# jrkerns/pylinac

Hardware: AMD Instinct MI355X
Metric: EPID images/s, filter->threshold->profile->peak on 1024^2 batch (higher is better)
Workload: dtype f64

## Files before the change

### pylinac_amd/csrc/gaussian_mm.hip

```cpp
#include <type_traits>

#include "pl_common.h"

namespace {

constexpr int kMmHalo = 24;
constexpr int kMmMaxRad = 24;

typedef int v4i __attribute__((ext_vector_type(4)));

constexpr int kMmDigits = 5;
constexpr int kMmQ = 40;

struct MmParams {
  unsigned band[kMmDigits][4][24];
  int c1;
  int c4;
  int radius;
  double wd[kMmMaxRad + 1];
};

bool mm_make_params(const double* h_wts , int R, MmParams& p) {
  if (R < 1 || R > kMmMaxRad) return false;
  double wmax = 0.0, W = 0.0;
  for (int k = 0; k <= 2 * R; ++k) {
    if (!(h_wts[k] >= 0.0)) return false;
    wmax = h_wts[k] > wmax ? h_wts[k] : wmax;
    W += h_wts[k];
  }
  if (!(wmax > 0.0) || !(W < 2.0)) return false;
  constexpr int Q = kMmQ;
  if (__builtin_ldexp(wmax, Q) >= 5.0e11) return false;
  long long wq[2 * kMmMaxRad + 1];
  long long WQ = 0;
  double eq = 0.0;
  signed char dig[kMmDigits][kMmMaxRad + 1];
  for (int k = 0; k <= 2 * R; ++k) {
    wq[k] = (long long)__builtin_llround(__builtin_ldexp(h_wts[k], Q));
    WQ += wq[k];
    eq += __builtin_fabs(h_wts[k] - __builtin_ldexp((double)wq[k], -Q));
  }
  for (int j = 0; j <= R; ++j) {
    if (wq[R - j] != wq[R + j]) return false;
    long long v = wq[R - j];
    for (int d = 0; d < kMmDigits; ++d) {
      const long long lo = ((v + 128) & 255) - 128;
      dig[d][j] = (signed char)lo;
      v = (v - lo) >> 8;
    }
    if (v != 0) return false;
  }
  for (int d = 0; d < kMmDigits; ++d)
    for (int c = 0; c < 4; ++c) {
      unsigned char bytes[96];
      for (int x = 0; x < 96; ++x) {
        const int pidx = x + c - 39;
        const int dist = pidx < 0 ? -pidx : pidx;
        bytes[x] = dist <= R ? (unsigned char)dig[d][dist] : 0;
      }
      for (int q = 0; q < 24; ++q)
        p.band[d][c][q] = (unsigned)bytes[4 * q] | ((unsigned)bytes[4 * q + 1] << 8) | ((unsigned)bytes[4 * q + 2] << 16) |
                          ((unsigned)bytes[4 * q + 3] << 24);
    }
  const double D = __builtin_ldexp(65535.0 * eq * (1.0 + 1e-9) + 65536.0 * __builtin_fabs(W - 1.0) + 1e-9, Q) +
                   (double)(2 * R + 1) * 16384.0 + 256.0;
  constexpr long long M = 1LL << 23;
  if (!(D < (double)M)) return false;
  const long long C = 32896LL * WQ + M;
  p.c1 = (int)((C & 0xffffffffLL) >> 8);
  p.c4 = (int)(C >> 32);
  p.radius = R;
  for (int j = 0; j <= kMmMaxRad; ++j) p.wd[j] = j <= R ? h_wts[R - j] : 0.0;
  return true;
}

__device__ __forceinline__ v4i mm_band_operand(const MmParams& P, int d, int lane) {
  const int p0 = 16 * (lane >> 4) - (lane & 15) + 15;
  const unsigned* src = &P.band[d][p0 & 3][p0 >> 2];
  return v4i{(int)src[0], (int)src[1], (int)src[2], (int)src[3]};
}

template <typename F>
__device__ __forceinline__ double mm_exact(F raw , const MmParams& P) {
  const int R = P.radius;
  double a = raw(0) * P.wd[0];
  for (int j = R; j >= 1; --j) a = __builtin_fma(raw(-j) + raw(j), P.wd[j], a);
  const double off = __builtin_fabs(__builtin_amdgcn_fract(__builtin_fabs(a)) - 0.5);
  if (off > 0.5 - 4e-9) {
    a = raw(0) * P.wd[0];
    for (int j = R; j >= 1; --j) a = a + (raw(-j) + raw(j)) * P.wd[j];
  }
  return a;
}

struct MmAcc { v4i v, z; };

struct MmConst { v4i c1, c4; };
__device__ __forceinline__ MmConst mm_const(const MmParams& P) {
  return MmConst{v4i{P.c1, P.c1, P.c1, P.c1}, v4i{P.c4, P.c4, P.c4, P.c4}};
}

template <bool IMG_IS_A>
__device__ __forceinline__ MmAcc mm_tile(v4i img_lo, v4i img_hi, const v4i (&w)[kMmDigits], const MmConst& K) {
  auto mm = [&](v4i img, v4i band, v4i c) -> v4i {
    return IMG_IS_A ? __builtin_amdgcn_mfma_i32_16x16x64_i8(img, band, c, 0, 0, 0)
                    : __builtin_amdgcn_mfma_i32_16x16x64_i8(band, img, c, 0, 0, 0);
  };
  v4i t = mm(img_lo, w[1], K.c1);
  t = mm(img_hi, w[0], t);
  t = mm(img_lo, w[2], t >> 8);
  t = mm(img_hi, w[1], t);
  v4i t3 = mm(img_lo, w[3], t >> 8);
  t3 = mm(img_hi, w[2], t3);
  v4i t4 = mm(img_lo, w[4], (t3 >> 8) + K.c4);
  t4 = mm(img_hi, w[3], t4);
  MmAcc r;
  r.v = mm(img_hi, w[4], t4 >> 8);
  r.z = (t3 | t4) & 255;
  return r;
}

template <bool IMG_IS_A, int NT>
__device__ __forceinline__ void mm_tiles(const v4i (&lo)[NT], const v4i (&hi)[NT], const v4i (&w)[kMmDigits], const MmConst& K,
                                         MmAcc (&r)[NT]) {
  auto mm = [&](v4i img, v4i band, v4i c) -> v4i {
    return IMG_IS_A ? __builtin_amdgcn_mfma_i32_16x16x64_i8(img, band, c, 0, 0, 0)
                    : __builtin_amdgcn_mfma_i32_16x16x64_i8(band, img, c, 0, 0, 0);
  };
  v4i t[NT], t3[NT], t4[NT];
#pragma unroll
  for (int i = 0; i < NT; ++i) t[i] = mm(lo[i], w[1], K.c1);
#pragma unroll
  for (int i = 0; i < NT; ++i) t[i] = mm(hi[i], w[0], t[i]);
#pragma unroll
  for (int i = 0; i < NT; ++i) t[i] = mm(lo[i], w[2], t[i] >> 8);
#pragma unroll
  for (int i = 0; i < NT; ++i) t[i] = mm(hi[i], w[1], t[i]);
#pragma unroll
  for (int i = 0; i < NT; ++i) t3[i] = mm(lo[i], w[3], t[i] >> 8);
#pragma unroll
  for (int i = 0; i < NT; ++i) t3[i] = mm(hi[i], w[2], t3[i]);
#pragma unroll
  for (int i = 0; i < NT; ++i) t4[i] = mm(lo[i], w[4], (t3[i] >> 8) + K.c4);
#pragma unroll
  for (int i = 0; i < NT; ++i) t4[i] = mm(hi[i], w[3], t4[i]);
#pragma unroll
  for (int i = 0; i < NT; ++i) {
    r[i].v = mm(hi[i], w[4], t4[i] >> 8);
    r[i].z = (t3[i] | t4[i]) & 255;
  }
}

template <bool SIGNED>
__device__ __forceinline__ double mm_value(unsigned char lo, unsigned char hi) {
  const int x = ((int)(signed char)hi + 128) * 256 + ((int)(signed char)lo + 128);
  return (double)(x - (SIGNED ? 32768 : 0));
}

constexpr int kFCols = 256;
constexpr int kFWin = kFCols + 2 * kMmHalo;
constexpr int kFPlane = kFWin * 16;
constexpr int kFQuadPitch = (kFWin / 4) * 16;

__device__ __forceinline__ int f_cell(int c) { return kFQuadPitch * (c & 3) + 16 * (c >> 2); }

struct FQuad { uint2 r[4]; };

__device__ __forceinline__ uint4 f_ldsq(const unsigned char* p) {
  return *reinterpret_cast<const uint4*>(p);
}

__device__ __forceinline__ void mm_set(uint2& res, int q, unsigned v16) {
  unsigned d = q < 2 ? res.x : res.y;
  d = (q & 1) ? (d & 0x0000ffffu) | (v16 << 16) : (d & 0xffff0000u) | v16;
  if (q < 2) res.x = d; else res.y = d;
}

__device__ __forceinline__ bool mm_wave_flat(const uint4& lo, const uint4& hi) {
  const unsigned l0 = lo.x, h0 = hi.x;
  const unsigned lf = __builtin_amdgcn_readfirstlane(l0), hf = __builtin_amdgcn_readfirstlane(h0);
  const unsigned d = (lo.y ^ l0) | (lo.z ^ l0) | (lo.w ^ l0) | (hi.y ^ h0) | (hi.z ^ h0) | (hi.w ^ h0) |
                     (__builtin_amdgcn_alignbit(l0, l0, 8) ^ l0) | (__builtin_amdgcn_alignbit(h0, h0, 8) ^ h0) | (lf ^ l0) | (hf ^ h0);
  return __ballot(d != 0u) == 0ull;
}

template <bool SIGNED>
__device__ __forceinline__ uint2 mm_finish_flag(const MmAcc& r, bool& bad) {
  unsigned v[4], z[4];
#pragma unroll
  for (int q = 0; q < 4; ++q) {
    v[q] = (unsigned)r.v[q];
    z[q] = (unsigned)r.z[q];
    if (SIGNED) v[q] = (v[q] + (v[q] < 32768u ? 1u : 0u)) ^ 0x8000u;
  }
  unsigned zm = z[0] < z[1] ? z[0] : z[1];
  zm = zm < z[2] ? zm : z[2];
  zm = zm < z[3] ? zm : z[3];
  bad = zm == 0u;
  return uint2{__builtin_amdgcn_perm(v[1], v[0], 0x05040100u), __builtin_amdgcn_perm(v[3], v[2], 0x05040100u)};
}

constexpr int kGThreads = 512;
constexpr int kGWaves = kGThreads / PL_WAVE;
constexpr int kGSlots = 5;
constexpr int kGInLo = 0;
constexpr int kGInHi = kGInLo + kGSlots * kFPlane;
constexpr int kGVLo = kGInHi + kGSlots * kFPlane;
constexpr int kGVHi = kGVLo + 2 * kFPlane;
constexpr int kGLds = kGVHi + 2 * kFPlane;

template <typename T>
__global__ void __launch_bounds__(kGThreads) __attribute__((amdgpu_waves_per_eu(4, 4)))
gauss2d_mm(const T* __restrict__ in, T* __restrict__ out, int h, int w, int strips, int segs, int seg_rows, const MmParams P) {
  constexpr bool kSigned = (T)-1 < (T)0;
  constexpr unsigned kHiFlip = kSigned ? 0u : 0x80808080u;
  __shared__ __attribute__((aligned(16))) unsigned char s_mem[kGLds];

  unsigned id = pl_xcd_remap(blockIdx.x, gridDim.x);
  const int ct = id % strips;
  id /= strips;
  const int rt = id % segs;
  const size_t frame = id / segs;
  const int tid = threadIdx.x;
  const int lane = tid & (PL_WAVE - 1);
  const int wave = __builtin_amdgcn_readfirstlane(tid / PL_WAVE);
  const int j = lane & 15, g = lane >> 4;
  const int c0 = ct * kFCols, r_begin = rt * seg_rows;
  const int r_end = r_begin + seg_rows < h ? r_begin + seg_rows : h;
  const int nsteps = (r_end - r_begin + 15) / 16;
  if (nsteps <= 0) return;
  const T* f = in + frame * (size_t)h * w;
  const int wcols = w - c0 < kFCols ? w - c0 : kFCols;
  const int nht = (wcols + 15) / 16;
  const int nvt = nht + 3;
  const bool ragged = (wcols & 15) != 0;
  const __amdgpu_buffer_rsrc_t src = pl_make_rsrc_bounded(f, (unsigned)h * (unsigned)w * 2u);
  const __amdgpu_buffer_rsrc_t dstb = pl_make_rsrc_bounded(out + (frame * (size_t)h + r_begin) * w, (unsigned)(r_end - r_begin) * (unsigned)w * 2u);

  const int rq = g;
  const int cqx = wave < 4 ? 16 * wave + j : 64 + j;
  const bool loader = (wave < 4 || (wave == 4 && j < 12)) && 4 * cqx < 16 * nvt;
  const int col0 = c0 - kMmHalo + 4 * cqx;
  const bool mir = col0 < 0 || col0 >= w;
  const int mc = col0 < 0 ? -col0 - 4 : (col0 >= w ? 2 * w - 4 - col0 : col0);
  const bool across = col0 < w && col0 + 4 > w;
  const unsigned colb = 2u * (unsigned)mc;
  const unsigned colb_ld = across ? colb - 4u : colb;
  const int qd0 = 16 * cqx + 4 * rq + (mir ? 3 * kFQuadPitch : 0);
  const int qdstep = mir ? -kFQuadPitch : kFQuadPitch;
  const unsigned wb = 2u * (unsigned)w;
  auto load_quad = [&](int k, FQuad& x) {
    const int rbase = r_begin - kMmHalo + 16 * k + 4 * rq;
#pragma unroll
    for (int i = 0; i < 4; ++i) {
      int r = rbase + i;
      r ^= r >> 31;
      const int r2 = 2 * h - 1 - r;
      r = r < r2 ? r : r2;
      x.r[i] = pl_buffer_load_u64(src, loader ? (unsigned)r * wb + colb_ld : 0x80000000u, 0);
    }
  };
  const bool any_across = (w & 3) == 2;
  auto store_quad = [&](int slot, const FQuad& xin) {
    if (!loader) return;
    FQuad x = xin;
    if (any_across) {
#pragma unroll
      for (int i = 0; i < 4; ++i) {
        const unsigned up = xin.r[i].y;
        x.r[i].x = across ? up : xin.r[i].x;
        x.r[i].y = across ? __builtin_amdgcn_alignbit(up, up, 16) : up;
      }
    }
    unsigned char* base = s_mem + kGInLo + slot * kFPlane + qd0;
#pragma unroll
    for (int half = 0; half < 2; ++half) {
      const unsigned a0 = half ? x.r[0].y : x.r[0].x, a1 = half ? x.r[1].y : x.r[1].x;
      const unsigned a2 = half ? x.r[2].y : x.r[2].x, a3 = half ? x.r[3].y : x.r[3].x;
      const unsigned e0 = __builtin_amdgcn_perm(a1, a0, 0x05010400u);
      const unsigned e1 = __builtin_amdgcn_perm(a3, a2, 0x05010400u);
      const unsigned o0 = __builtin_amdgcn_perm(a1, a0, 0x07030602u);
      const unsigned o1 = __builtin_amdgcn_perm(a3, a2, 0x07030602u);
      unsigned char* pe = base + (2 * half) * qdstep;
      unsigned char* po = base + (2 * half + 1) * qdstep;
      *reinterpret_cast<unsigned*>(pe) = __builtin_amdgcn_perm(e1, e0, 0x05040100u) ^ 0x80808080u;
      *reinterpret_cast<unsigned*>(pe + (kGInHi - kGInLo)) = __builtin_amdgcn_perm(e1, e0, 0x07060302u) ^ kHiFlip;
      *reinterpret_cast<unsigned*>(po) = __builtin_amdgcn_perm(o1, o0, 0x05040100u) ^ 0x80808080u;
      *reinterpret_cast<unsigned*>(po + (kGInHi - kGInLo)) = __builtin_amdgcn_perm(o1, o0, 0x07060302u) ^ kHiFlip;
    }
  };
  v4i band[kMmDigits];
#pragma unroll
  for (int d = 0; d < kMmDigits; ++d) band[d] = mm_band_operand(P, d, lane);
  __builtin_amdgcn_s_waitcnt(0x0f70);
  MmConst K = mm_const(P);
  asm volatile("" : "+v"(K.c1), "+v"(K.c4));
  FQuad nxt;
  {
    FQuad a[4];
#pragma unroll
    for (int k = 0; k < 4; ++k) load_quad(k, a[k]);
    load_quad(4, nxt);
#pragma unroll
    for (int k = 0; k < 4; ++k) store_quad(k, a[k]);
  }
  __syncthreads();

  const int lane_cell = f_cell(j);
  int slot_g = g;
  int wslot = 4;
  auto step = [&](int s) {
    const int vb = (s & 1) * kFPlane;
    const int lrow = 16 * s + j;
    const bool row_ok = r_begin + lrow < r_end;

    {
      const unsigned char* ain = s_mem + kGInLo + slot_g * kFPlane + lane_cell;
      unsigned char* vout = s_mem + kGVLo + vb + 16 * j + 4 * g;
      auto run = [&](auto NT, int t0, int tstep) {
        constexpr int N = decltype(NT)::value;
        auto tile_of = [&](int i) { const int t = t0 + tstep * i; return t < nvt ? t : 0; };
        unsigned badbits = 0;
        v4i lo[N], hi[N];
#pragma unroll
        for (int i = 0; i < N; ++i) {
          const uint4 qlo = f_ldsq(ain + 64 * tile_of(i));
          const uint4 qhi = f_ldsq(ain + 64 * tile_of(i) + (kGInHi - kGInLo));
          lo[i] = v4i{(int)qlo.x, (int)qlo.y, (int)qlo.z, (int)qlo.w};
          hi[i] = v4i{(int)qhi.x, (int)qhi.y, (int)qhi.z, (int)qhi.w};
        }
        MmAcc acc[N];
        mm_tiles<true, N>(lo, hi, band, K, acc);
#pragma unroll
        for (int i = 0; i < N; ++i) {
          bool bad;
          const uint2 res = mm_finish_flag<kSigned>(acc[i], bad);
          badbits |= (bad && row_ok) ? (1u << i) : 0u;
          unsigned char* vd = vout + 256 * tile_of(i);
          *reinterpret_cast<unsigned*>(vd) = __builtin_amdgcn_perm(res.y, res.x, 0x06040200u) ^ 0x80808080u;
          *reinterpret_cast<unsigned*>(vd + (kGVHi - kGVLo)) = __builtin_amdgcn_perm(res.y, res.x, 0x07050301u) ^ kHiFlip;
        }
        if (__ballot(badbits != 0u) == 0ull) return;
        auto sample = [&](int x, int p) {
          const int a = ((s + (p >> 4)) % kGSlots) * kFPlane + f_cell(x) + (p & 15);
          return mm_value<kSigned>(s_mem[kGInLo + a], s_mem[kGInHi + a]);
        };
#pragma unroll 1
        for (int i = 0; i < N; ++i) {
          if (__ballot((badbits >> i) & 1u) == 0ull) continue;
          const int t = tile_of(i);
          unsigned char* vd = vout + 256 * t;
          const uint4 flo = *reinterpret_cast<const uint4*>(ain + 64 * t);
          const uint4 fhi = *reinterpret_cast<const uint4*>(ain + 64 * t + (kGInHi - kGInLo));
          if (mm_wave_flat(flo, fhi)) {
            const double c = sample(16 * t, 0);
            const unsigned v = (unsigned short)pl_from_double<T>(mm_exact([&](int) { return c; }, P));
            *reinterpret_cast<unsigned*>(vd) = (0x01010101u * (v & 255u)) ^ 0x80808080u;
            *reinterpret_cast<unsigned*>(vd + (kGVHi - kGVLo)) = (0x01010101u * (v >> 8)) ^ kHiFlip;
          } else {
            const MmAcc ra = mm_tile<true>(v4i{(int)flo.x, (int)flo.y, (int)flo.z, (int)flo.w}, v4i{(int)fhi.x, (int)fhi.y, (int)fhi.z, (int)fhi.w}, band, K);
            if ((badbits >> i) & 1u) {
#pragma unroll 1
              for (int q = 0; q < 4; ++q) {
                if (ra.z[q] != 0) continue;
                const int x = 16 * t + 4 * g + q;
                const unsigned v = (unsigned short)pl_from_double<T>(mm_exact([&](int k) { return sample(x, kMmHalo + j + k); }, P));
                vd[q] = (unsigned char)((v & 255u) ^ 0x80u);
                vd[q + (kGVHi - kGVLo)] = (unsigned char)((v >> 8) ^ (kHiFlip & 0x80u));
              }
            }
          }
        }
      };
      if (wave < 5) run(std::integral_constant<int, 2>{}, wave, 5); else run(std::integral_constant<int, 3>{}, 5 + wave, 3);
    }
    store_quad(wslot, nxt);
    load_quad(s + 5, nxt);
    __syncthreads();

    {
      const unsigned char* bin = s_mem + kGVLo + vb + 16 * j + 256 * g;
      const unsigned doff = row_ok ? ((unsigned)lrow * (unsigned)w + (unsigned)(c0 + 4 * g)) * 2u : 0x80000000u;
      const unsigned doff16 = row_ok ? ((unsigned)lrow * (unsigned)w + (unsigned)(c0 + 8 * (g >> 1))) * 2u : 0x80000000u;
      auto store_cut = [&](unsigned off, int x0, unsigned d0, unsigned d1, unsigned d2, unsigned d3) {
        const unsigned d[4] = {d0, d1, d2, d3};
#pragma unroll
        for (int k = 0; k < 4; ++k) pl_buffer_store_u32(d[k], dstb, x0 + 2 * k < wcols ? off + 4u * (unsigned)k : 0x80000000u, 0);
      };
      auto tile_of = [&](int i) { const int t = 2 * wave + i; return t < nht ? t : 0; };
      constexpr int N = 2;
      unsigned badbits = 0;
      auto hpass = [&](auto RAGGED) {
        v4i lo[N], hi[N];
#pragma unroll
        for (int i = 0; i < N; ++i) {
          const uint4 qlo = f_ldsq(bin + 256 * tile_of(i));
          const uint4 qhi = f_ldsq(bin + 256 * tile_of(i) + (kGVHi - kGVLo));
          lo[i] = v4i{(int)qlo.x, (int)qlo.y, (int)qlo.z, (int)qlo.w};
          hi[i] = v4i{(int)qhi.x, (int)qhi.y, (int)qhi.z, (int)qhi.w};
        }
        MmAcc acc[N];
        mm_tiles<false, N>(lo, hi, band, K, acc);
        bool bad0, bad1;
        const uint2 r0 = mm_finish_flag<kSigned>(acc[0], bad0), r1 = mm_finish_flag<kSigned>(acc[1], bad1);
        badbits |= ((bad0 && row_ok) ? 1u : 0u) | ((bad1 && row_ok) ? 2u : 0u);
        const auto sx = __builtin_amdgcn_permlane16_swap(r0.x, r1.x, false, false);
        const auto sy = __builtin_amdgcn_permlane16_swap(r0.y, r1.y, false, false);
        const unsigned tsel = (g & 1) ? (unsigned)tile_of(1) : (unsigned)tile_of(0);
        const uint4 piece{(unsigned)sx[0], (unsigned)sy[0], (unsigned)sx[1], (unsigned)sy[1]};
        if (!decltype(RAGGED)::value) {
          pl_buffer_store_u128(piece, dstb, doff16 + 32u * tsel, 0);
        } else {
          store_cut(doff16 + 32u * tsel, 16 * (int)tsel + 8 * (g >> 1), piece.x, piece.y, piece.z, piece.w);
        }
      };
      if (ragged) hpass(std::true_type{}); else hpass(std::false_type{});
      if (__ballot(badbits != 0u) != 0ull) {
        __builtin_amdgcn_s_waitcnt(0x0f70);
        auto store_cut2 = [&](unsigned off, int x0, unsigned d0, unsigned d1) {
          pl_buffer_store_u32(d0, dstb, x0 < wcols ? off : 0x80000000u, 0);
          pl_buffer_store_u32(d1, dstb, x0 + 2 < wcols ? off + 4u : 0x80000000u, 0);
        };
        auto sample = [&](int row, int x) {
          const int a = vb + 256 * (x >> 4) + 16 * row + (x & 15);
          return mm_value<kSigned>(s_mem[kGVLo + a], s_mem[kGVHi + a]);
        };
#pragma unroll 1
        for (int i = 0; i < N; ++i) {
          if (__ballot((badbits >> i) & 1u) == 0ull) continue;
          const int t = tile_of(i);
          const uint4 flo = *reinterpret_cast<const uint4*>(bin + 256 * t);
          const uint4 fhi = *reinterpret_cast<const uint4*>(bin + 256 * t + (kGVHi - kGVLo));
          if (mm_wave_flat(flo, fhi)) {
            const double c = sample(0, 16 * t);
            const unsigned v = (unsigned short)pl_from_double<T>(mm_exact([&](int) { return c; }, P));
            store_cut2(doff + 32u * (unsigned)t, 16 * t + 4 * g, v | (v << 16), v | (v << 16));
          } else {
            const MmAcc ra = mm_tile<false>(v4i{(int)flo.x, (int)flo.y, (int)flo.z, (int)flo.w}, v4i{(int)fhi.x, (int)fhi.y, (int)fhi.z, (int)fhi.w}, band, K);
            if ((badbits >> i) & 1u) {
              bool dummy;
              uint2 res = mm_finish_flag<kSigned>(ra, dummy);
#pragma unroll 1
              for (int q = 0; q < 4; ++q) {
                if (ra.z[q] != 0) continue;
                const int x = kMmHalo + 16 * t + 4 * g + q;
                mm_set(res, q, (unsigned short)pl_from_double<T>(mm_exact([&](int k) { return sample(j, x + k); }, P)));
              }
              store_cut2(doff + 32u * (unsigned)t, 16 * t + 4 * g, res.x, res.y);
            }
          }
        }
      }
    }
    slot_g = slot_g == kGSlots - 1 ? 0 : slot_g + 1;
    wslot = wslot == kGSlots - 1 ? 0 : wslot + 1;
  };
#pragma unroll 1
  for (int s = 0; s < nsteps; ++s) step(s);
}


template <typename T>
int launch_mm2d_t(const T* in, T* out, int64_t n, int h, int w, const MmParams& P, hipStream_t st) {
  const int strips = (int)pl_cdiv(w, kFCols);
  const int64_t resident = (int64_t)pl_cu_count() * 2;
  const int64_t max_segs = h / 128 > 1 ? h / 128 : 1;
  int64_t segs = 1, best = -1;
  for (int64_t cand = 1; cand <= max_segs; ++cand) {
    const int64_t rows = pl_cdiv(pl_cdiv(h, cand), 16) * 16;
    const int64_t wgs = n * strips * pl_cdiv(h, rows);
    const int64_t cost = pl_cdiv(wgs, resident) * (rows / 16 + 3);
    if (best < 0 || cost < best) { best = cost; segs = cand; }
  }
  const int seg_rows = (int)(pl_cdiv(pl_cdiv(h, segs), 16) * 16);
  segs = pl_cdiv(h, seg_rows);
  const int64_t blocks = n * strips * segs;
  if (blocks > 0x7fffffffLL) return -1;
  hipLaunchKernelGGL(gauss2d_mm<T>, dim3((unsigned)blocks), dim3(kGThreads), 0, st, in, out, h, w, strips, (int)segs, seg_rows, P);
  return 0;
}

}

int pl_gauss_mm2d_covers(const void* in, const void* out, int h, int w, int radius) {
  if (radius < 1 || radius > kMmMaxRad || h < 64 || w < 64 || (w & 1) || (int64_t)h * w * 2 >= 0x7fff0000LL) return 0;
  return !((reinterpret_cast<uintptr_t>(in) & 3) || (reinterpret_cast<uintptr_t>(out) & 3));
}

int pl_gauss_mm2d_launch(const void* in, void* out, int is_signed, int64_t n, int h, int w, const double* wts, int radius,
                         hipStream_t st) {
  if (!pl_gauss_mm2d_covers(in, out, h, w, radius)) return -1;
  MmParams P;
  if (!mm_make_params(wts, radius, P)) return -1;
  return is_signed ? launch_mm2d_t<short>((const short*)in, (short*)out, n, h, w, P, st)
                   : launch_mm2d_t<unsigned short>((const unsigned short*)in, (unsigned short*)out, n, h, w, P, st);
}
```

### pylinac_amd/csrc/pl_common.h

```cpp
#pragma once
#include <hip/hip_runtime.h>
#include <stdint.h>

#include <atomic>

#include "../../include/pylinac_hip.h"

#define PL_WAVE 64

void pl_set_error(const char* fmt, ...);
int pl_check_launch(const char* what);

#define PL_REQUIRE(cond, msg)                    \
  do {                                           \
    if (!(cond)) {                               \
      pl_set_error("%s: %s", __func__, msg);     \
      return PL_ERR_INVALID_ARG;                 \
    }                                            \
  } while (0)

static inline int64_t pl_cdiv(int64_t a, int64_t b) { return (a + b - 1) / b; }

int pl_cu_count();

struct PlPackbitsGeom {
  const int64_t* expect;
  const int64_t* dst;
  const int32_t* status_index;
};
int64_t pl_packbits_work_bytes(int64_t n_streams, int64_t max_stream_bytes);
void pl_packbits_expand(const unsigned char* d_bytes, int64_t nbytes, const int64_t* d_off, const int64_t* d_len,
                        int64_t n_streams, int64_t max_stream_bytes, unsigned char* d_out, int32_t* d_status,
                        unsigned char* d_work, PlPackbitsGeom geom, hipStream_t st);

int64_t pl_adler32_slots_bytes(int64_t n_ranges, int64_t max_len);
void pl_adler32_launch(const unsigned char* d_bytes, int64_t nbytes, const int64_t* d_off, const int64_t* d_len, int64_t n_ranges,
                       int64_t max_len, const int32_t* d_gate, const uint32_t* d_expected, int mismatch, uint32_t* d_adler,
                       int32_t* d_status, unsigned char* d_slots, hipStream_t st);

struct PnChecked {
  uint32_t* trailer;
  int32_t* judge;
  int64_t* in_used;
  int64_t max_out;
  int overflow;
};
void pl_inflate_launch(bool checked, const unsigned char* d_bytes, int64_t nbytes, const int64_t* d_in_off, const int64_t* d_in_len,
                       int64_t n_streams, int wrapper, unsigned char* d_out, const int64_t* d_out_off, const int64_t* d_out_cap,
                       int64_t* d_out_len, int32_t* d_status, PnChecked chk, hipStream_t st);

__device__ __forceinline__ int pl_reflect(int i, int n) {
  if ((unsigned)i < (unsigned)n) return i;
  const int m1 = (i < 0) ? (-i - 1) : (2 * n - 1 - i);
  if ((unsigned)m1 < (unsigned)n) return m1;
  const int p = 2 * n;
  int m = i % p;
  if (m < 0) m += p;
  return m >= n ? p - 1 - m : m;
}

__device__ __forceinline__ unsigned pl_umed3(unsigned a, unsigned b, unsigned c) {
  unsigned r;
  asm("v_med3_u32 %0, %1, %2, %3" : "=v"(r) : "v"(a), "v"(b), "v"(c));
  return r;
}
__device__ __forceinline__ int pl_smed3(int a, int b, int c) {
  int r;
  asm("v_med3_i32 %0, %1, %2, %3" : "=v"(r) : "v"(a), "v"(b), "v"(c));
  return r;
}

__device__ __forceinline__ unsigned pl_xcd_remap(unsigned b, unsigned nwg) {
  unsigned q = nwg >> 3, r = nwg & 7u, xcd = b & 7u;
  unsigned base = xcd < r ? xcd * (q + 1) : r * (q + 1) + (xcd - r) * q;
  return base + (b >> 3);
}

template <typename T>
__device__ __forceinline__ T pl_from_double(double v);
template <>
__device__ __forceinline__ unsigned short pl_from_double<unsigned short>(double v) {
  return (unsigned short)(unsigned int)v;
}
template <>
__device__ __forceinline__ short pl_from_double<short>(double v) {
  return (short)(int)v;
}
template <>
__device__ __forceinline__ float pl_from_double<float>(double v) {
  return (float)v;
}
template <>
__device__ __forceinline__ double pl_from_double<double>(double v) {
  return v;
}
template <>
__device__ __forceinline__ int pl_from_double<int>(double v) {
  return (int)v;
}
template <>
__device__ __forceinline__ long long pl_from_double<long long>(double v) {
  return (long long)v;
}
template <>
__device__ __forceinline__ unsigned char pl_from_double<unsigned char>(double v) {
  return (unsigned char)(unsigned int)v;
}

__device__ __forceinline__ __amdgpu_buffer_rsrc_t pl_make_rsrc(const void* base) {
  return __builtin_amdgcn_make_buffer_rsrc(const_cast<void*>(base), 0, -1, 0x00020000);
}
__device__ __forceinline__ unsigned pl_buffer_load_u32(__amdgpu_buffer_rsrc_t r, unsigned lane_off, unsigned uniform_off) {
  return (unsigned)__builtin_amdgcn_raw_buffer_load_b32(r, (int)lane_off, (int)uniform_off, 0);
}
__device__ __forceinline__ void pl_buffer_store_u32(unsigned v, __amdgpu_buffer_rsrc_t r, unsigned lane_off,
                                                    unsigned uniform_off) {
  __builtin_amdgcn_raw_buffer_store_b32(v, r, (int)lane_off, (int)uniform_off, 0);
}

__device__ __forceinline__ __amdgpu_buffer_rsrc_t pl_make_rsrc_bounded(const void* base, unsigned bytes) {
  return __builtin_amdgcn_make_buffer_rsrc(const_cast<void*>(base), 0, (int)bytes, 0x00020000);
}
__device__ __forceinline__ uint2 pl_buffer_load_u64(__amdgpu_buffer_rsrc_t r, unsigned lane_off, unsigned uniform_off) {
  const auto v = __builtin_amdgcn_raw_buffer_load_b64(r, (int)lane_off, (int)uniform_off, 0);
  return uint2{(unsigned)v[0], (unsigned)v[1]};
}
__device__ __forceinline__ void pl_buffer_store_u64(uint2 v, __amdgpu_buffer_rsrc_t r, unsigned lane_off, unsigned uniform_off) {
  typedef unsigned pl_v2u __attribute__((ext_vector_type(2)));
  __builtin_amdgcn_raw_buffer_store_b64(pl_v2u{v.x, v.y}, r, (int)lane_off, (int)uniform_off, 0);
}

__device__ __forceinline__ void pl_buffer_store_u128(uint4 v, __amdgpu_buffer_rsrc_t r, unsigned lane_off, unsigned uniform_off) {
  typedef unsigned pl_v4u __attribute__((ext_vector_type(4)));
  __builtin_amdgcn_raw_buffer_store_b128(pl_v4u{v.x, v.y, v.z, v.w}, r, (int)lane_off, (int)uniform_off, 0);
}
__device__ __forceinline__ uint4 pl_buffer_load_u128(__amdgpu_buffer_rsrc_t r, unsigned lane_off, unsigned uniform_off) {
#ifdef PL_HIPEMU
  const uint2 a = pl_buffer_load_u64(r, lane_off, uniform_off), b = pl_buffer_load_u64(r, lane_off + 8u, uniform_off);
  return uint4{a.x, a.y, b.x, b.y};
#else
  const auto v = __builtin_amdgcn_raw_buffer_load_b128(r, (int)lane_off, (int)uniform_off, 0);
  return uint4{(unsigned)v[0], (unsigned)v[1], (unsigned)v[2], (unsigned)v[3]};
#endif
}
__device__ __forceinline__ unsigned pl_buffer_load_u16(__amdgpu_buffer_rsrc_t r, unsigned lane_off, unsigned uniform_off) {
#ifdef PL_HIPEMU
  const unsigned d = pl_buffer_load_u32(r, lane_off & ~3u, uniform_off);
  return (lane_off & 2u) ? d >> 16 : d & 0xffffu;
#else
  return (unsigned)__builtin_amdgcn_raw_buffer_load_b16(r, (int)lane_off, (int)uniform_off, 0);
#endif
}
template <typename T>
__device__ __forceinline__ int pl_extend16_here(int v) {
  unsigned short e = (unsigned short)v;
  asm volatile("" : "+v"(e));
  return (int)(T)e;
}
constexpr unsigned kPlBufferNowhere = 0x80000000u;

__device__ __forceinline__ int pl_wave_from_prev(int v) { return __builtin_amdgcn_update_dpp(v, v, 0x138, 0xf, 0xf, false); }
__device__ __forceinline__ int pl_wave_from_next(int v) { return __builtin_amdgcn_update_dpp(v, v, 0x130, 0xf, 0xf, false); }

struct PlQuot {
  double s, d, r;
  bool fast;
};
__device__ __forceinline__ PlQuot pl_quot_make(double s, double d) {
  PlQuot k;
  k.s = s;
  k.d = d;
  k.fast = d >= 1.0 && d <= 65535.0 && d == floor(d) && s >= 0.0 && s <= 65535.0 && s == floor(s);
  k.r = k.fast ? 1.0 / d : 0.0;
  return k;
}
__device__ __forceinline__ double pl_quot(const PlQuot& k, double a) {
  const double x = a - k.s;
  if (k.fast) {
    const double q0 = x * k.r;
    const double rem = fma(-q0, k.d, x);
    return fma(rem, k.r, q0);
  }
  return x / k.d;
}

typedef __attribute__((address_space(3))) unsigned pl_lds_u32;
__device__ __forceinline__ void pl_lds_add_abs(unsigned byte_addr, unsigned v) {
  __hip_atomic_fetch_add((pl_lds_u32*)(uintptr_t)byte_addr, v, __ATOMIC_RELAXED, __HIP_MEMORY_SCOPE_WORKGROUP);
}
__device__ __forceinline__ unsigned pl_lds_base(const void* lds_ptr) { return (unsigned)reinterpret_cast<uintptr_t>(lds_ptr); }

#define PL_CONSTANT_AS __attribute__((address_space(4)))
template <typename T>
__device__ __forceinline__ const PL_CONSTANT_AS T* pl_constant_ptr(const T* p) {
  return (const PL_CONSTANT_AS T*)p;
}

__device__ __forceinline__ void pl_wave_sync() {
  __builtin_amdgcn_fence(__ATOMIC_RELEASE, "wavefront");
  __builtin_amdgcn_wave_barrier();
  __builtin_amdgcn_fence(__ATOMIC_ACQUIRE, "wavefront");
}

__device__ __forceinline__ double pl_readlane_f64(double v, int l) {
  const long long b = __double_as_longlong(v);
  const int lo = __builtin_amdgcn_readlane((int)b, l), hi = __builtin_amdgcn_readlane((int)(b >> 32), l);
  return __longlong_as_double((long long)(((unsigned long long)(unsigned)hi << 32) | (unsigned long long)(unsigned)lo));
}

template <typename T, typename F>
__device__ __forceinline__ T pl_wave_reduce(T v, F f) {
#pragma unroll
  for (int o = 32; o > 0; o >>= 1) v = f(v, __shfl_xor(v, o, 64));
  return v;
}

template <int CTRL, int RM>
__device__ __forceinline__ int pl_dpp_keep(int v) { return __builtin_amdgcn_update_dpp(v, v, CTRL, RM, 0xf, false); }

template <typename F>
__device__ __forceinline__ int pl_wave_reduce_idem(int v, F f) {
  v = f(v, pl_dpp_keep<0x111, 0xf>(v));
  v = f(v, pl_dpp_keep<0x112, 0xf>(v));
  v = f(v, pl_dpp_keep<0x114, 0xf>(v));
  v = f(v, pl_dpp_keep<0x118, 0xf>(v));
  v = f(v, pl_dpp_keep<0x142, 0xa>(v));
  v = f(v, pl_dpp_keep<0x143, 0xc>(v));
  return __builtin_amdgcn_readlane(v, 63);
}
template <typename F>
__device__ __forceinline__ double pl_wave_reduce_idem(double v, F f) {
  auto step = [&](auto tag_lo, auto tag_hi) {
    const long long b = __double_as_longlong(v);
    const int lo = tag_lo((int)b), hi = tag_hi((int)(b >> 32));
    v = f(v, __longlong_as_double((long long)(((unsigned long long)(unsigned)hi << 32) | (unsigned long long)(unsigned)lo)));
  };
  step([](int x) { return pl_dpp_keep<0x111, 0xf>(x); }, [](int x) { return pl_dpp_keep<0x111, 0xf>(x); });
  step([](int x) { return pl_dpp_keep<0x112, 0xf>(x); }, [](int x) { return pl_dpp_keep<0x112, 0xf>(x); });
  step([](int x) { return pl_dpp_keep<0x114, 0xf>(x); }, [](int x) { return pl_dpp_keep<0x114, 0xf>(x); });
  step([](int x) { return pl_dpp_keep<0x118, 0xf>(x); }, [](int x) { return pl_dpp_keep<0x118, 0xf>(x); });
  step([](int x) { return pl_dpp_keep<0x142, 0xa>(x); }, [](int x) { return pl_dpp_keep<0x142, 0xa>(x); });
  step([](int x) { return pl_dpp_keep<0x143, 0xc>(x); }, [](int x) { return pl_dpp_keep<0x143, 0xc>(x); });
  return pl_readlane_f64(v, 63);
}

__device__ __forceinline__ unsigned pl_group8_sum(unsigned v) {
  v += (unsigned)__builtin_amdgcn_update_dpp(0, (int)v, 0xB1, 0xf, 0xf, true);
  v += (unsigned)__builtin_amdgcn_update_dpp(0, (int)v, 0x4E, 0xf, 0xf, true);
  v += (unsigned)__builtin_amdgcn_update_dpp(0, (int)v, 0x141, 0xf, 0xf, true);
  return v;
}
__device__ __forceinline__ unsigned long long pl_group8_sum(unsigned long long v) {
  auto from = [](unsigned long long x, auto mv) {
    return ((unsigned long long)(unsigned)mv((int)(x >> 32)) << 32) | (unsigned long long)(unsigned)mv((int)x);
  };
  v += from(v, [](int x) { return __builtin_amdgcn_update_dpp(0, x, 0xB1, 0xf, 0xf, true); });
  v += from(v, [](int x) { return __builtin_amdgcn_update_dpp(0, x, 0x4E, 0xf, 0xf, true); });
  v += from(v, [](int x) { return __builtin_amdgcn_update_dpp(0, x, 0x141, 0xf, 0xf, true); });
  return v;
}

__device__ __forceinline__ unsigned pl_group8_max(unsigned v) {
  v = max(v, (unsigned)__builtin_amdgcn_update_dpp(0, (int)v, 0xB1, 0xf, 0xf, true));
  v = max(v, (unsigned)__builtin_amdgcn_update_dpp(0, (int)v, 0x4E, 0xf, 0xf, true));
  v = max(v, (unsigned)__builtin_amdgcn_update_dpp(0, (int)v, 0x141, 0xf, 0xf, true));
  return v;
}

#define PL_DISPATCH_DTYPE(dtype, T, ...)                         \
  switch (dtype) {                                               \
    case PL_U16: { using T = unsigned short; __VA_ARGS__; break; } \
    case PL_I16: { using T = short; __VA_ARGS__; break; }        \
    case PL_F32: { using T = float; __VA_ARGS__; break; }        \
    case PL_F64: { using T = double; __VA_ARGS__; break; }       \
    case PL_U8: { using T = unsigned char; __VA_ARGS__; break; } \
    case PL_I32: { using T = int; __VA_ARGS__; break; }          \
    case PL_I64: { using T = long long; __VA_ARGS__; break; }    \
    default:                                                     \
      pl_set_error("%s: unsupported dtype %d", __func__, (int)(dtype)); \
      return PL_ERR_UNSUPPORTED;                                 \
  }
```

Baseline: 370,100.

## Fold level-4 bias constant into unsigned path and add interior fast-path loads

Replaces the runtime c4 bias operand with a compile-time constant, and for unsigned inputs removes it from the MFMA chain entirely by compensating with packed 16-bit adds on the output pixels. The bad-pixel flag is reworked to carry per-tile zero minima, so the ballot is computed from a single reduced value. The row loader gains an interior fast path that issues unconditional buffer loads when the whole 16-row quad lies inside the image, skipping the per-row reflect logic. The parameter builder now rejects weight sets whose high constant bits differ from the fixed bias, which narrows the set of kernels the MFMA path accepts.

```diff
diff --git a/pylinac_amd/csrc/gaussian_mm.hip b/pylinac_amd/csrc/gaussian_mm.hip
--- a/pylinac_amd/csrc/gaussian_mm.hip
+++ b/pylinac_amd/csrc/gaussian_mm.hip
@@ -11,11 +11,11 @@
 
 constexpr int kMmDigits = 5;
 constexpr int kMmQ = 40;
+constexpr long long kMmBias = 32896;
 
 struct MmParams {
   unsigned band[kMmDigits][4][24];
   int c1;
-  int c4;
   int radius;
   double wd[kMmMaxRad + 1];
 };
@@ -67,8 +67,9 @@
   constexpr long long M = 1LL << 23;
   if (!(D < (double)M)) return false;
   const long long C = 32896LL * WQ + M;
-  p.c1 = (int)((C & 0xffffffffLL) >> 8);
-  p.c4 = (int)(C >> 32);
+  const long long Chi = C >> kMmQ, Clo = C - (Chi << kMmQ);
+  if (Chi != kMmBias || Clo >= (1LL << 32)) return false;
+  p.c1 = (int)(Clo >> 8);
   p.radius = R;
   for (int j = 0; j <= kMmMaxRad; ++j) p.wd[j] = j <= R ? h_wts[R - j] : 0.0;
   return true;
@@ -95,12 +96,17 @@
 
 struct MmAcc { v4i v, z; };
 
-struct MmConst { v4i c1, c4; };
+struct MmConst { v4i c1; };
 __device__ __forceinline__ MmConst mm_const(const MmParams& P) {
-  return MmConst{v4i{P.c1, P.c1, P.c1, P.c1}, v4i{P.c4, P.c4, P.c4, P.c4}};
-}
-
-template <bool IMG_IS_A>
+  return MmConst{v4i{P.c1, P.c1, P.c1, P.c1}};
+}
+template <bool FOLD>
+__device__ __forceinline__ v4i mm_level4(v4i t3) {
+  constexpr int kC4 = (int)(kMmBias * 256);
+  return FOLD ? t3 >> 8 : (t3 >> 8) + v4i{kC4, kC4, kC4, kC4};
+}
+
+template <bool IMG_IS_A, bool FOLD>
 __device__ __forceinline__ MmAcc mm_tile(v4i img_lo, v4i img_hi, const v4i (&w)[kMmDigits], const MmConst& K) {
   auto mm = [&](v4i img, v4i band, v4i c) -> v4i {
     return IMG_IS_A ? __builtin_amdgcn_mfma_i32_16x16x64_i8(img, band, c, 0, 0, 0)
@@ -112,7 +118,7 @@
   t = mm(img_hi, w[1], t);
   v4i t3 = mm(img_lo, w[3], t >> 8);
   t3 = mm(img_hi, w[2], t3);
-  v4i t4 = mm(img_lo, w[4], (t3 >> 8) + K.c4);
+  v4i t4 = mm(img_lo, w[4], mm_level4<FOLD>(t3));
   t4 = mm(img_hi, w[3], t4);
   MmAcc r;
   r.v = mm(img_hi, w[4], t4 >> 8);
@@ -120,7 +126,7 @@
   return r;
 }
 
-template <bool IMG_IS_A, int NT>
+template <bool IMG_IS_A, bool FOLD, int NT>
 __device__ __forceinline__ void mm_tiles(const v4i (&lo)[NT], const v4i (&hi)[NT], const v4i (&w)[kMmDigits], const MmConst& K,
                                          MmAcc (&r)[NT]) {
   auto mm = [&](v4i img, v4i band, v4i c) -> v4i {
@@ -141,7 +147,7 @@
 #pragma unroll
   for (int i = 0; i < NT; ++i) t3[i] = mm(hi[i], w[2], t3[i]);
 #pragma unroll
-  for (int i = 0; i < NT; ++i) t4[i] = mm(lo[i], w[4], (t3[i] >> 8) + K.c4);
+  for (int i = 0; i < NT; ++i) t4[i] = mm(lo[i], w[4], mm_level4<FOLD>(t3[i]));
 #pragma unroll
   for (int i = 0; i < NT; ++i) t4[i] = mm(hi[i], w[3], t4[i]);
 #pragma unroll
@@ -185,7 +191,7 @@
 }
 
 template <bool SIGNED>
-__device__ __forceinline__ uint2 mm_finish_flag(const MmAcc& r, bool& bad) {
+__device__ __forceinline__ uint2 mm_finish_flag(const MmAcc& r, unsigned& zmin) {
   unsigned v[4], z[4];
 #pragma unroll
   for (int q = 0; q < 4; ++q) {
@@ -195,9 +201,23 @@
   }
   unsigned zm = z[0] < z[1] ? z[0] : z[1];
   zm = zm < z[2] ? zm : z[2];
-  zm = zm < z[3] ? zm : z[3];
-  bad = zm == 0u;
+  zmin = zm < z[3] ? zm : z[3];
   return uint2{__builtin_amdgcn_perm(v[1], v[0], 0x05040100u), __builtin_amdgcn_perm(v[3], v[2], 0x05040100u)};
+}
+template <bool SIGNED>
+__device__ __forceinline__ uint2 mm_pixels(uint2 res) {
+  return SIGNED ? res : uint2{pl_pk_add_u16(res.x, 0x80808080u), pl_pk_add_u16(res.y, 0x80808080u)};
+}
+template <bool SIGNED>
+__device__ __forceinline__ void mm_store_planes(unsigned char* vd, int hi_off, uint2 res) {
+  if (SIGNED) {
+    *reinterpret_cast<unsigned*>(vd) = __builtin_amdgcn_perm(res.y, res.x, 0x06040200u) ^ 0x80808080u;
+    *reinterpret_cast<unsigned*>(vd + hi_off) = __builtin_amdgcn_perm(res.y, res.x, 0x07050301u);
+  } else {
+    *reinterpret_cast<unsigned*>(vd) = __builtin_amdgcn_perm(res.y, res.x, 0x06040200u);
+    *reinterpret_cast<unsigned*>(vd + hi_off) =
+        __builtin_amdgcn_perm(pl_pk_add_u16(res.y, 0x00800080u), pl_pk_add_u16(res.x, 0x00800080u), 0x07050301u);
+  }
 }
 
 constexpr int kGThreads = 512;
@@ -214,6 +234,7 @@
 gauss2d_mm(const T* __restrict__ in, T* __restrict__ out, int h, int w, int strips, int segs, int seg_rows, const MmParams P) {
   constexpr bool kSigned = (T)-1 < (T)0;
   constexpr unsigned kHiFlip = kSigned ? 0u : 0x80808080u;
+  constexpr bool kFold = !kSigned;
   __shared__ __attribute__((aligned(16))) unsigned char s_mem[kGLds];
 
   unsigned id = pl_xcd_remap(blockIdx.x, gridDim.x);
@@ -249,8 +270,15 @@
   const int qd0 = 16 * cqx + 4 * rq + (mir ? 3 * kFQuadPitch : 0);
   const int qdstep = mir ? -kFQuadPitch : kFQuadPitch;
   const unsigned wb = 2u * (unsigned)w;
-  auto load_quad = [&](int k, FQuad& x) {
-    const int rbase = r_begin - kMmHalo + 16 * k + 4 * rq;
+  const unsigned off_in = loader ? 4u * (unsigned)rq * wb + colb_ld : 0x80000000u;
+  auto load_quad = [&](int k, FQuad& x, bool may_be_inside) {
+    const int rb0 = r_begin - kMmHalo + 16 * k;
+    if (may_be_inside && rb0 >= 0 && rb0 + 16 <= h) {
+#pragma unroll
+      for (int i = 0; i < 4; ++i) x.r[i] = pl_buffer_load_u64(src, off_in, (unsigned)(rb0 + i) * wb);
+      return;
+    }
+    const int rbase = rb0 + 4 * rq;
 #pragma unroll
     for (int i = 0; i < 4; ++i) {
       int r = rbase + i;
@@ -294,13 +322,13 @@
   for (int d = 0; d < kMmDigits; ++d) band[d] = mm_band_operand(P, d, lane);
   __builtin_amdgcn_s_waitcnt(0x0f70);
   MmConst K = mm_const(P);
-  asm volatile("" : "+v"(K.c1), "+v"(K.c4));
+  asm volatile("" : "+v"(K.c1));
   FQuad nxt;
   {
     FQuad a[4];
 #pragma unroll
-    for (int k = 0; k < 4; ++k) load_quad(k, a[k]);
-    load_quad(4, nxt);
+    for (int k = 0; k < 4; ++k) load_quad(k, a[k], false);
+    load_quad(4, nxt, false);
 #pragma unroll
     for (int k = 0; k < 4; ++k) store_quad(k, a[k]);
   }
@@ -320,7 +348,6 @@
       auto run = [&](auto NT, int t0, int tstep) {
         constexpr int N = decltype(NT)::value;
         auto tile_of = [&](int i) { const int t = t0 + tstep * i; return t < nvt ? t : 0; };
-        unsigned badbits = 0;
         v4i lo[N], hi[N];
 #pragma unroll
         for (int i = 0; i < N; ++i) {
@@ -330,17 +357,18 @@
           hi[i] = v4i{(int)qhi.x, (int)qhi.y, (int)qhi.z, (int)qhi.w};
         }
         MmAcc acc[N];
-        mm_tiles<true, N>(lo, hi, band, K, acc);
+        mm_tiles<true, kFold, N>(lo, hi, band, K, acc);
+        unsigned zm[N], zall = 0u;
 #pragma unroll
         for (int i = 0; i < N; ++i) {
-          bool bad;
-          const uint2 res = mm_finish_flag<kSigned>(acc[i], bad);
-          badbits |= (bad && row_ok) ? (1u << i) : 0u;
-          unsigned char* vd = vout + 256 * tile_of(i);
-          *reinterpret_cast<unsigned*>(vd) = __builtin_amdgcn_perm(res.y, res.x, 0x06040200u) ^ 0x80808080u;
-          *reinterpret_cast<unsigned*>(vd + (kGVHi - kGVLo)) = __builtin_amdgcn_perm(res.y, res.x, 0x07050301u) ^ kHiFlip;
+          const uint2 res = mm_finish_flag<kSigned>(acc[i], zm[i]);
+          zall = (i == 0 || zm[i] < zall) ? zm[i] : zall;
+          mm_store_planes<kSigned>(vout + 256 * tile_of(i), kGVHi - kGVLo, res);
         }
-        if (__ballot(badbits != 0u) == 0ull) return;
+        if (__ballot(zall == 0u && row_ok) == 0ull) return;
+        unsigned badbits = 0;
+#pragma unroll
+        for (int i = 0; i < N; ++i) badbits |= (zm[i] == 0u && row_ok) ? (1u << i) : 0u;
         auto sample = [&](int x, int p) {
           const int a = ((s + (p >> 4)) % kGSlots) * kFPlane + f_cell(x) + (p & 15);
           return mm_value<kSigned>(s_mem[kGInLo + a], s_mem[kGInHi + a]);
@@ -358,7 +386,7 @@
             *reinterpret_cast<unsigned*>(vd) = (0x01010101u * (v & 255u)) ^ 0x80808080u;
             *reinterpret_cast<unsigned*>(vd + (kGVHi - kGVLo)) = (0x01010101u * (v >> 8)) ^ kHiFlip;
           } else {
-            const MmAcc ra = mm_tile<true>(v4i{(int)flo.x, (int)flo.y, (int)flo.z, (int)flo.w}, v4i{(int)fhi.x, (int)fhi.y, (int)fhi.z, (int)fhi.w}, band, K);
+            const MmAcc ra = mm_tile<true, kFold>(v4i{(int)flo.x, (int)flo.y, (int)flo.z, (int)flo.w}, v4i{(int)fhi.x, (int)fhi.y, (int)fhi.z, (int)fhi.w}, band, K);
             if ((badbits >> i) & 1u) {
 #pragma unroll 1
               for (int q = 0; q < 4; ++q) {
@@ -375,7 +403,7 @@
       if (wave < 5) run(std::integral_constant<int, 2>{}, wave, 5); else run(std::integral_constant<int, 3>{}, 5 + wave, 3);
     }
     store_quad(wslot, nxt);
-    load_quad(s + 5, nxt);
+    load_quad(s + 5, nxt, true);
     __syncthreads();
 
     {
@@ -389,7 +417,7 @@
       };
       auto tile_of = [&](int i) { const int t = 2 * wave + i; return t < nht ? t : 0; };
       constexpr int N = 2;
-      unsigned badbits = 0;
+      unsigned zm0, zm1;
       auto hpass = [&](auto RAGGED) {
         v4i lo[N], hi[N];
 #pragma unroll
@@ -400,10 +428,9 @@
           hi[i] = v4i{(int)qhi.x, (int)qhi.y, (int)qhi.z, (int)qhi.w};
         }
         MmAcc acc[N];
-        mm_tiles<false, N>(lo, hi, band, K, acc);
-        bool bad0, bad1;
-        const uint2 r0 = mm_finish_flag<kSigned>(acc[0], bad0), r1 = mm_finish_flag<kSigned>(acc[1], bad1);
-        badbits |= ((bad0 && row_ok) ? 1u : 0u) | ((bad1 && row_ok) ? 2u : 0u);
+        mm_tiles<false, kFold, N>(lo, hi, band, K, acc);
+        const uint2 r0 = mm_pixels<kSigned>(mm_finish_flag<kSigned>(acc[0], zm0));
+        const uint2 r1 = mm_pixels<kSigned>(mm_finish_flag<kSigned>(acc[1], zm1));
         const auto sx = __builtin_amdgcn_permlane16_swap(r0.x, r1.x, false, false);
         const auto sy = __builtin_amdgcn_permlane16_swap(r0.y, r1.y, false, false);
         const unsigned tsel = (g & 1) ? (unsigned)tile_of(1) : (unsigned)tile_of(0);
@@ -415,7 +442,8 @@
         }
       };
       if (ragged) hpass(std::true_type{}); else hpass(std::false_type{});
-      if (__ballot(badbits != 0u) != 0ull) {
+      if (__ballot((zm0 < zm1 ? zm0 : zm1) == 0u && row_ok) != 0ull) {
+        const unsigned badbits = ((zm0 == 0u && row_ok) ? 1u : 0u) | ((zm1 == 0u && row_ok) ? 2u : 0u);
         __builtin_amdgcn_s_waitcnt(0x0f70);
         auto store_cut2 = [&](unsigned off, int x0, unsigned d0, unsigned d1) {
           pl_buffer_store_u32(d0, dstb, x0 < wcols ? off : 0x80000000u, 0);
@@ -436,10 +464,10 @@
             const unsigned v = (unsigned short)pl_from_double<T>(mm_exact([&](int) { return c; }, P));
             store_cut2(doff + 32u * (unsigned)t, 16 * t + 4 * g, v | (v << 16), v | (v << 16));
           } else {
-            const MmAcc ra = mm_tile<false>(v4i{(int)flo.x, (int)flo.y, (int)flo.z, (int)flo.w}, v4i{(int)fhi.x, (int)fhi.y, (int)fhi.z, (int)fhi.w}, band, K);
+            const MmAcc ra = mm_tile<false, kFold>(v4i{(int)flo.x, (int)flo.y, (int)flo.z, (int)flo.w}, v4i{(int)fhi.x, (int)fhi.y, (int)fhi.z, (int)fhi.w}, band, K);
             if ((badbits >> i) & 1u) {
-              bool dummy;
-              uint2 res = mm_finish_flag<kSigned>(ra, dummy);
+              unsigned dummy;
+              uint2 res = mm_pixels<kSigned>(mm_finish_flag<kSigned>(ra, dummy));
 #pragma unroll 1
               for (int q = 0; q < 4; ++q) {
                 if (ra.z[q] != 0) continue;
@@ -487,6 +515,11 @@
   return !((reinterpret_cast<uintptr_t>(in) & 3) || (reinterpret_cast<uintptr_t>(out) & 3));
 }
 
+int pl_gauss_mm2d_taps_covered(const double* wts, int radius) {
+  MmParams P;
+  return mm_make_params(wts, radius, P) ? 1 : 0;
+}
+
 int pl_gauss_mm2d_launch(const void* in, void* out, int is_signed, int64_t n, int h, int w, const double* wts, int radius,
                          hipStream_t st) {
   if (!pl_gauss_mm2d_covers(in, out, h, w, radius)) return -1;
diff --git a/pylinac_amd/csrc/pl_common.h b/pylinac_amd/csrc/pl_common.h
--- a/pylinac_amd/csrc/pl_common.h
+++ b/pylinac_amd/csrc/pl_common.h
@@ -57,6 +57,15 @@
   int m = i % p;
   if (m < 0) m += p;
   return m >= n ? p - 1 - m : m;
+}
+
+__device__ __forceinline__ unsigned pl_pk_add_u16(unsigned a, unsigned b) {
+#ifdef PL_HIPEMU
+  return ((a & 0x7fff7fffu) + (b & 0x7fff7fffu)) ^ ((a ^ b) & 0x80008000u);
+#else
+  typedef unsigned short pl_v2u16 __attribute__((ext_vector_type(2)));
+  return __builtin_bit_cast(unsigned, (pl_v2u16)(__builtin_bit_cast(pl_v2u16, a) + __builtin_bit_cast(pl_v2u16, b)));
+#endif
 }
 
 __device__ __forceinline__ unsigned pl_umed3(unsigned a, unsigned b, unsigned c) {
```

Result: faster. 377,700, median of 6 (+2.1%).
